# aatifjiwani/lens-flare

Hardware: AMD Instinct MI355X
Metric: Mray-surface-intersections/s + frame time, 1080p 256spp double-Gauss (higher is better)
Workload: dtype f32

## Files before the change

### lens-flare_amd/csrc/lf_api.hip

```cpp
#include <algorithm>
#include <cmath>
#include <cstdio>
#include <cstdlib>
#include <cstring>

#include "lf_internal.h"
#include "lf_march_events.h"
#include "../host/lf_collada.h"

lf_status lf_fail(const lf_ctx* ctx, lf_status st, const std::string& msg) {
  if (ctx) ctx->err = msg;
  return st;
}

static constexpr size_t kTimedCap = 512;

static hipEvent_t timing_event(lf_ctx* ctx) {
  if (!ctx->event_pool.empty()) {
    hipEvent_t e = ctx->event_pool.back();
    ctx->event_pool.pop_back();
    return e;
  }
  hipEvent_t e = nullptr;
  if (hipEventCreate(&e) != hipSuccess) return nullptr;
// ... 158 lines not shown
  ctx->lenscam_dirty = true;
  if (grow2) return lfk_mask_support(ctx);
  return LF_OK;
}

}

void lf_coat_constants(float n, float m, float np, float thickness_nm, float lambda_nm, LfCoatK* c) {
  const float m2 = m * m, n2 = n * n, np2 = np * np;
  c->dm = m2 - n2;
  c->ph = (2.0f * thickness_nm) / lambda_nm;
  c->s01 = 1.0f / (n + m);
  c->s12 = 1.0f / (m + np);
  const float q1 = std::fmaf(m2, n, n2 * m), q2 = std::fmaf(np2, m, m2 * np);
  c->p01a = m2 / q1; c->p01b = n2 / q1;
  c->p12a = np2 / q2; c->p12b = m2 / q2;
}

extern "C" {

int lf_abi_version(void) { return LF_ABI_VERSION; }

const char* lf_last_error(const lf_ctx* ctx) { return ctx ? ctx->err.c_str() : "null context"; }

static std::mutex g_knob_mu;
static std::vector<std::pair<std::string, double>> g_knob_defaults;

lf_status lf_create(lf_ctx** out, int device) {
  if (!out) return LF_ERR_INVALID;
  *out = nullptr;
  int n = 0;
  if (hipGetDeviceCount(&n) != hipSuccess || n <= 0) return LF_ERR_NO_DEVICE;
  if (device < 0 || device >= n) return LF_ERR_NO_DEVICE;
  if (hipSetDevice(device) != hipSuccess) return LF_ERR_NO_DEVICE;
  {
    hipDeviceProp_t prop;
    if (hipGetDeviceProperties(&prop, device) != hipSuccess) return LF_ERR_NO_DEVICE;
    bool any_arch = false;
#ifdef LF_EXPERIMENTS
    any_arch = std::getenv("LF_ALLOW_ANY_ARCH") != nullptr;
#endif
    if (std::strncmp(prop.gcnArchName, "gfx950", 6) != 0 && !any_arch) return LF_ERR_NO_DEVICE;
  }
  lf_ctx* ctx = new lf_ctx();
  ctx->device = device;
  if (hipStreamCreateWithFlags(&ctx->stream, hipStreamNonBlocking) != hipSuccess) {
    delete ctx;
    return LF_ERR_HIP;
  }
  ctx->own_stream = true;
#ifdef LF_EXPERIMENTS
  if (const char* sb = std::getenv("LF_MARCH_SUB_BITS")) {
    int v = std::atoi(sb);
    if (v >= 0 && v <= 8) ctx->march_sub_bits = v;
  }
#endif
  default_paraxial_lens(ctx->pl);
  bool ok = hipMalloc((void**)&ctx->flares, sizeof(LfFlares)) == hipSuccess &&
            hipMalloc((void**)&ctx->ghosts, sizeof(LfGhostList)) == hipSuccess &&
            hipMalloc((void**)&ctx->pl_dev, sizeof(LfParaxialLens)) == hipSuccess &&
            hipMalloc((void**)&ctx->lens_dev, sizeof(LfLensDev)) == hipSuccess &&
            hipMalloc((void**)&ctx->pairs_dev, sizeof(LfPairsDev)) == hipSuccess &&
            hipMalloc((void**)&ctx->counters_dev, kMarchCounterSlots * sizeof(unsigned long long)) == hipSuccess &&
            hipMalloc((void**)&ctx->scene_counters_dev, kSceneCounters * sizeof(unsigned long long)) == hipSuccess &&
            hipMalloc((void**)&ctx->primary_dev, sizeof(LfPrimaryDev)) == hipSuccess;
  for (int s = 0; s < 2 && ok; s++)
    ok = hipMalloc((void**)&ctx->ap[s].stats, sizeof(lf_aperture_stats)) == hipSuccess;
  if (!ok) { lf_destroy(ctx); return LF_ERR_OOM; }
  (void)hipMemset(ctx->flares, 0, sizeof(LfFlares));
  (void)hipMemset(ctx->ghosts, 0, sizeof(LfGhostList));
  (void)hipMemset(ctx->counters_dev, 0, kMarchCounterSlots * sizeof(unsigned long long));
  (void)hipMemset(ctx->scene_counters_dev, 0, kSceneCounters * sizeof(unsigned long long));
  if (upload_paraxial(ctx) != LF_OK) { lf_destroy(ctx); return LF_ERR_HIP; }
  {
    std::vector<std::pair<std::string, double>> defaults;
    { std::lock_guard<std::mutex> lock(g_knob_mu); defaults = g_knob_defaults; }
    for (const auto& kv : defaults) (void)lf_test_knob(ctx, kv.first.c_str(), kv.second);
  }
  *out = ctx;
  return LF_OK;
}

lf_status lf_destroy(lf_ctx* ctx) {
  if (!ctx) return LF_ERR_INVALID;
  if (ctx->comm_poisoned.load() && ctx->comm_busy.load() > 0) return LF_ERR_STATE;
  (void)hipSetDevice(ctx->device);
  (void)hipDeviceSynchronize();
  (void)lf_comm_destroy(ctx);
  if (ctx->comm_stage) (void)hipFree(ctx->comm_stage);
  free_frame_buffers(ctx);
  lf_cull_cache_free(ctx);
  for (auto& t : ctx->timed) { (void)hipEventDestroy(t.start); (void)hipEventDestroy(t.stop); }
  for (hipEvent_t e : ctx->event_pool) (void)hipEventDestroy(e);
  for (int s = 0; s < 2; s++) {
    if (ctx->ap[s].texels) (void)hipFree(ctx->ap[s].texels);
    if (ctx->ap[s].stats) (void)hipFree(ctx->ap[s].stats);
  }
  void* ptrs[] = {ctx->spectrum, ctx->twiddle, ctx->dft_rows, ctx->flares, ctx->ghosts, ctx->pl_dev,
                  ctx->lens_dev, ctx->pairs_dev, ctx->counters_dev, ctx->accum,
                  ctx->prog_dev, ctx->sun_lights_dev,
                  ctx->scene_dev.nodes, ctx->scene_dev.prims, ctx->scene_dev.normals, ctx->scene_dev.materials,
                  ctx->scene_dev.lights, ctx->env_block, ctx->probe_dev, ctx->scene_counters_dev,
                  ctx->primary_dev, ctx->cull_dev, ctx->cull_lists.list[0], ctx->cull_lists.list[1], ctx->cull_counts, ctx->cull_popc_dev,
                  ctx->tail_acc, ctx->tail_done};
  for (void* p : ptrs) if (p) (void)hipFree(p);
  if (ctx->own_stream && ctx->stream) (void)hipStreamDestroy(ctx->stream);
  delete ctx;
// ... 537 lines not shown
  LF_HIP(ctx, hipMemcpy(&f, ctx->flares, sizeof(f), hipMemcpyDeviceToHost));
  if (flare >= f.n_flares) return lf_fail(ctx, LF_ERR_INVALID, "lf_set_sun_from_flares: no such flare in the frame");
  if (!(efl_mm > 0.0)) {
    if (!paraxial_image_scale(ctx->raw_n, ctx->raw_stop, ctx->raw_radius, ctx->raw_thickness,
                              ctx->raw_ior + (size_t)(ctx->lens.n_lambda / 2) * ctx->raw_n, &efl_mm) || !(efl_mm > 0.0))
      return lf_fail(ctx, LF_ERR_INVALID, "lf_set_sun_from_flares: the prescription images no distant point on its sensor");
  }
  const double sw = ctx->sensor_w_mm, sh = sw * (double)ctx->H / (double)ctx->W;
  const float dir[3] = {(float)((f.origin[flare][0] - 0.5) * sw / efl_mm),
                        (float)((f.origin[flare][1] - 0.5) * sh / efl_mm), -1.0f};
  const float rad[3] = {(float)f.radiance[flare][0], (float)f.radiance[flare][1], (float)f.radiance[flare][2]};
  return lf_set_sun(ctx, dir, rad, angular_radius);
}

lf_status lf_set_ghost_pairs(lf_ctx* ctx, const int* pairs, int n_pairs, int include_primary) {
  if (!ctx || n_pairs < 0) return LF_ERR_INVALID;
  if (!ctx->lens_valid) return lf_fail(ctx, LF_ERR_STATE, "lf_set_ghost_pairs before lf_set_lens");
  LfPairsDev P;
  std::memset(&P, 0, sizeof(P));
  const int ns = ctx->lens.n_surf, stop = ctx->lens.stop;
  if (include_primary) { P.ij[P.n][0] = -1; P.ij[P.n][1] = -1; P.n++; }
  if (!pairs || n_pairs == 0) {
    for (int i = 0; i < ns; i++)
      for (int j = i + 1; j < ns; j++) {
        if (i == stop || j == stop) continue;
        if (P.n >= LF_MAX_PAIRS + 1) return lf_fail(ctx, LF_ERR_INVALID, "too many ghost pairs");
        P.ij[P.n][0] = i; P.ij[P.n][1] = j; P.n++;
      }
  } else {
    if (n_pairs > LF_MAX_PAIRS) return lf_fail(ctx, LF_ERR_INVALID, "too many ghost pairs");
    for (int q = 0; q < n_pairs; q++) {
      int i = pairs[2 * q], j = pairs[2 * q + 1];
      if (i == -1 && j == -1) {
        if (P.n > 0 && P.ij[0][0] < 0) return lf_fail(ctx, LF_ERR_INVALID, "primary path listed twice");
        if (P.n > 0) {
          for (int k = P.n; k > 0; k--) { P.ij[k][0] = P.ij[k - 1][0]; P.ij[k][1] = P.ij[k - 1][1]; }
        }
        P.ij[0][0] = -1; P.ij[0][1] = -1; P.n++;
        continue;
      }
      if (i < 0 || j <= i || j >= ns || i == stop || j == stop)
        return lf_fail(ctx, LF_ERR_INVALID, "ghost pair must satisfy 0 <= i < j < n, neither the stop");
      P.ij[P.n][0] = i; P.ij[P.n][1] = j; P.n++;
    }
  }
  if (P.n == 0) return lf_fail(ctx, LF_ERR_INVALID, "empty pair set");
  ctx->pairs = P;
  ctx->events_dirty = true;
  return LF_OK;
}

lf_status lf_set_pupil_subcells(lf_ctx* ctx, int bits) {
  if (!ctx) return LF_ERR_INVALID;
  if (bits < 0 || bits > 8) return lf_fail(ctx, LF_ERR_INVALID, "pupil sub-cell bits must be 0..8");
  ctx->march_sub_bits = bits;
  return LF_OK;
}

lf_status lf_set_tile_stride(lf_ctx* ctx, int stride) {
  if (!ctx) return LF_ERR_INVALID;
  if (stride != 1 && stride != 2 && stride != 4 && stride != 8)
    return lf_fail(ctx, LF_ERR_INVALID, "tile stride must be 1, 2, 4 or 8");
  ctx->march_xstride_log2 = stride == 1 ? 0 : stride == 2 ? 1 : stride == 4 ? 2 : 3;
  return LF_OK;
}

lf_status lf_trace_ghosts(lf_ctx* ctx, int spp, uint64_t key) {
  if (!ctx || spp <= 0) return LF_ERR_INVALID;
  if (!ctx->lens_valid || !ctx->sun_valid)
    return lf_fail(ctx, LF_ERR_STATE, "lf_trace_ghosts needs lf_set_lens and lf_set_sun");
  if (!ctx->ap[LF_APERTURE_STARBURST].valid)
    return lf_fail(ctx, LF_ERR_STATE, "aperture mask (LF_APERTURE_STARBURST slot) not set");
  if (ctx->pupil_target_h > 0.0f && ctx->lens.stop >= 0) {
    for (int q = 0; q < ctx->pairs.n; q++)
      if (ctx->pairs.ij[q][0] > ctx->lens.stop)
        return lf_fail(ctx, LF_ERR_STATE,
                       "a pupil target is set and the pair selection holds a pair with both mirrors behind the stop: "
                       "such pairs need the default disc (march them in a second launch, lf_set_ghost_accumulate)");
  }
  LF_HIP(ctx, hipSetDevice(ctx->device));
  lf_status st = lfk_march(ctx, spp, key);
  if (st != LF_OK) return st;
  ctx->ghost_valid = true;
  return LF_OK;
}

lf_status lf_set_march_culling(lf_ctx* ctx, int mode) {
  if (!ctx) return LF_ERR_INVALID;
  if (mode < 0 || mode > 2) return lf_fail(ctx, LF_ERR_INVALID, "march culling: 0 off, 1 on, 2 on and rebuilt at every launch");
  ctx->march_cull = mode;
  return LF_OK;
}

lf_status lf_set_cull_share(lf_ctx* ctx, int rank, int nranks) {
  if (!ctx) return LF_ERR_INVALID;
  if (nranks < 1 || nranks > 64 || rank < 0 || rank >= nranks) return lf_fail(ctx, LF_ERR_INVALID, "lf_set_cull_share: 0 <= rank < nranks <= 64");
  if (ctx->split.table == LfSplit::kComm) return lf_fail(ctx, LF_ERR_STATE, "lf_set_cull_share: the table is shared through the communicator (lf_comm_share_cull)");
  if (nranks > 1 && ctx->split.deal == LfSplit::kBlocks)
    return lf_fail(ctx, LF_ERR_STATE, "lf_set_cull_share: the frame is dealt by blocks (lf_set_block_deal): every rank builds the rows it reads, nothing is shared");
  lf_install_split(ctx, nranks > 1 ? ctx->split.with_table(LfSplit::kHost, rank, nranks) : ctx->split.with_table(LfSplit::kOwn));
  return LF_OK;
}

lf_status lf_cull_prepare(lf_ctx* ctx, int spp) {
  if (!ctx) return LF_ERR_INVALID;
  if (ctx->split.table != LfSplit::kHost) return lf_fail(ctx, LF_ERR_STATE, "lf_cull_prepare without lf_set_cull_share(rank, nranks > 1)");
  if (!ctx->lens_valid || !ctx->ap[LF_APERTURE_STARBURST].valid || ctx->W == 0)
// ... 777 lines not shown
```

### lens-flare_amd/csrc/lf_cull.hip

```cpp
#include <algorithm>
#include <cstdio>
#include <cstdlib>

#include "lf_internal.h"
#include "lf_march_events.h"
#include "lf_march_common.h"

namespace {

using namespace lfm;

constexpr int kWgWaves = 8;
constexpr int kListMax = 4096;

struct PathTally {
  unsigned long long n_rays = 0, events = 0, n_clip = 0, n_vign = 0, n_tir = 0, n_scene = 0, n_rm_lane = 0, n_rm_rows = 0;
  unsigned long long executed = 0;
  unsigned n_light = 0;
};

__device__ __forceinline__ void march_channel_factors(const LfLensDev* __restrict__ lens, float* __restrict__ s_chan, int tid) {
  if (tid < LF_MAX_LAMBDA * 3) {
    const int l = tid / 3, c = tid - 3 * l;
    s_chan[tid] = l < lens->n_lambda ? lens->sun_radiance[c] * lens->lambda_rgb[l][c] : 0.0f;
  }
}

template <int K, bool W1, int VAR>
__device__ __forceinline__ void march_started_path(const LfLensDev* __restrict__ lens, const LfPairsDev* __restrict__ pairs,
                                                   const int* __restrict__ seq_table, const LfProgRow* __restrict__ rec_table,
                                                   const LfWeightRow* __restrict__ wrec_table, const float* __restrict__ mask,
                                                   const MarchArgs& a, int q, lanemask start_mask, float X, float Y,
                                                   const StartRay& s0, int lane, int acc_slot,
                                                   unsigned long long* __restrict__ s_acc, const float* __restrict__ s_chan,
                                                   PathTally& T) {
  const int n_lambda = lens->n_lambda, prog_recs = pairs->prog_recs;
  const int n_groups = (n_lambda + K - 1) / K;
  const float inv_stop_h = a.inv_stop_h, lobe_thr = a.lobe_thr;
  const float sx = lens->sun_dir[0], sy = lens->sun_dir[1], sz = lens->sun_dir[2];
  const float inv_1mc = lens->sun_inv_one_minus_cos, sun_ss = lens->sun_ss;
  const int n_ev = pairs->ev_cnt[q];
  const int* const seq = seq_table + pairs->ev_off[q];
  for (int g = 0; g < n_groups; g++) {
    const LfProgRow* const recs = rec_table + (size_t)g * (size_t)prog_recs;
    const LfWeightRow* const wrecs = wrec_table + (size_t)g * (size_t)prog_recs;
    Ray r[K];
    lanemask alive[K];
    unsigned nlive = 0u;
#pragma unroll
    for (int j = 0; j < K; j++) {
      r[j] = Ray{X, Y, 0.0f, fmaf(X, X, Y * Y), s0.dx, s0.dy, s0.dz, s0.w0, 1.0f};
      const float ns = lens->n_start[min(g * K + j, n_lambda - 1)];
      r[j].dx *= ns; r[j].dy *= ns; r[j].dz *= ns;
      alive[j] = (g * K + j < n_lambda) ? start_mask : 0ull;
      nlive += (unsigned)__popcll(alive[j]);
    }
    T.n_rays += nlive;
    unsigned ev32 = 0u;
    unsigned se = (unsigned)*(const int __attribute__((address_space(4)))*)(seq);
    int e = 0;
    if (n_ev > 0 && nlive != 0u) for (;;) {
      const unsigned cur = se;
      se = (unsigned)*(const int __attribute__((address_space(4)))*)(seq + e + 1);
      const LfProgRow wr = load_prec(recs, cur & 0xffffu);
      LfWeightRow ww;
      if (W1) ww = load_wrec(wrecs, cur & 0xffffu);
// ... 22 lines not shown
          for (int j = 0; j < K; j++) {
            if (K > 1 && __builtin_expect(alive[j] == 0ull, 0)) { okv[j] = 0ull; gv[j] = 0ull; continue; }
            okv[j] = surface_event<W1>(r[j], wr.dzv, wr.curv, wr.ch, wr.c2, wr.sc, wr.cn22[j], wr.rn2[j],
                                       wr.delta[j], wr.h2, false, false, wr.sgn, gv[j], ww.fs[j], ww.fo[j], ww.fi[j],
                                       CoatSel<VAR>{wrec_table, ww.coat, j});
            died |= alive[j] & ~okv[j];
          }
        } else if (kind == (unsigned)LF_EV_REFLECT) {
#pragma unroll
          for (int j = 0; j < K; j++) {
            if (K > 1 && __builtin_expect(alive[j] == 0ull, 0)) { okv[j] = 0ull; gv[j] = 0ull; continue; }
            okv[j] = surface_event<W1>(r[j], wr.dzv, wr.curv, wr.ch, wr.c2, wr.sc, wr.cn22[j], wr.rn2[j],
                                       wr.delta[j], wr.h2, true, false, wr.sgn, gv[j], ww.fs[j], ww.fo[j], ww.fi[j],
                                       CoatSel<VAR>{wrec_table, ww.coat, j});
            died |= alive[j] & ~okv[j];
          }
        } else {
#pragma unroll
          for (int j = 0; j < K; j++) {
            if (K > 1 && __builtin_expect(alive[j] == 0ull, 0)) { okv[j] = 0ull; gv[j] = 0ull; continue; }
            okv[j] = surface_event<W1>(r[j], wr.dzv, wr.curv, wr.ch, wr.c2, wr.sc, wr.cn22[j], wr.rn2[j],
                                       wr.delta[j], wr.h2, (kind & LF_EV_REFLECT) != 0, (kind & LF_EV_FLAT) != 0,
                                       wr.sgn, gv[j], ww.fs[j], ww.fo[j], ww.fi[j],
                                       CoatSel<VAR>{wrec_table, ww.coat, j});
            died |= alive[j] & ~okv[j];
          }
        }
        if (__builtin_expect(died != 0ull, 0)) {
#pragma unroll
          for (int j = 0; j < K; j++) {
            T.n_vign += (unsigned)__popcll(alive[j] & ~gv[j]);
            T.n_tir += (unsigned)__popcll(alive[j] & gv[j] & ~okv[j]);
            nlive -= (unsigned)__popcll(alive[j] & ~okv[j]);
            alive[j] &= okv[j];
          }
          if (nlive == 0u) e = n_ev;
        }
      }
      ev32 += nlive;
      if (++e >= n_ev) break;
    }
    T.events += ev32;
    T.executed += ev32;
    if (nlive == 0u) continue;
    T.n_scene += nlive;
    lanemask lit[K], lit_any = 0ull;
#pragma unroll
    for (int j = 0; j < K; j++) {
      const float cg = fmaf(r[j].dx, sx, fmaf(r[j].dy, sy, r[j].dz * sz));
      lit[j] = alive[j] & __ballot(cg > lobe_thr);
      lit_any |= lit[j];
    }
    if (lit_any == 0ull) continue;
    for (int j = 0; j < K; j++) {
      lanemask lj = lit[0];
#pragma unroll
      for (int jj = 1; jj < K; jj++) lj = (j == jj) ? lit[jj] : lj;
      if (lj == 0ull) continue;
      const int l = g * K + j;
      Ray rw = j == 0 ? r[0] : j == 1 ? r[K > 1 ? 1 : 0] : r[K > 2 ? 2 : 0];
      if (!W1) {
        rw = Ray{X, Y, 0.0f, fmaf(X, X, Y * Y), s0.dx, s0.dy, s0.dz, s0.w0, 1.0f};
        { const float ns = lens->n_start[l]; rw.dx *= ns; rw.dy *= ns; rw.dz *= ns; }
        T.n_rm_lane += (unsigned long long)((unsigned)n_ev * (unsigned)__popcll(lj));
        T.n_rm_rows += (unsigned)n_ev;
        weighted_remarch<VAR>(rw, seq, n_ev, j, recs, wrecs, wrec_table, mask, inv_stop_h, a.mw, a.mh);
      }
      const float qq = lobe_q(rw.dx, rw.dy, rw.dz, sx, sy, sz, sun_ss, inv_1mc);
      const float om = 1.0f - qq;
      float contrib = __fdiv_rn(rw.wn, rw.wd) * (om * om);
      contrib = (((lj >> lane) & 1ull) != 0ull && qq < 1.0f && contrib > 0.0f) ? contrib : 0.0f;
      T.n_light += contrib > 0.0f ? 1u : 0u;
#pragma unroll
      for (int c = 0; c < 3; c++) {
        const float v = contrib * s_chan[l * 3 + c];
        const unsigned long long fx = (unsigned long long)(v * 68719476736.0f);
        if (fx) atomicAdd(&s_acc[acc_slot * 3 + c], fx);
      }
    }
  }
}

template <int K, bool REFLECT, bool FLAT>
__device__ __forceinline__ lanemask surface_rows(Ray (&r)[K], const lanemask (&alive)[K], const LfProgRow& wr, lanemask (&okv)[K],
                                                 lanemask (&gv)[K]) {
  lanemask died = 0ull;
#pragma unroll
  for (int j = 0; j < K; j++) {
    if (K > 1 && __builtin_expect(alive[j] == 0ull, 0)) { okv[j] = 0ull; gv[j] = 0ull; continue; }
    okv[j] = surface_event<false>(r[j], wr.dzv, wr.curv, wr.ch, wr.c2, wr.sc, wr.cn22[j], wr.rn2[j], wr.delta[j], wr.h2,
                                  REFLECT, FLAT, wr.sgn, gv[j]);
    died |= alive[j] & ~okv[j];
  }
  return died;
}

template <int K, int VAR>
__device__ __forceinline__ void march_started_set(const LfLensDev* __restrict__ lens, const LfPairsDev* __restrict__ pairs,
                                                  const int* __restrict__ seq_table, const LfProgRow* __restrict__ rec_table,
                                                  const LfWeightRow* __restrict__ wrec_table, const float* __restrict__ mask,
                                                  const MarchArgs& a, unsigned long long todo, lanemask active_mask, float X, float Y,
                                                  const StartRay& s0, int lane, unsigned long long* __restrict__ s_acc,
                                                  const int2* __restrict__ s_meta, const float* __restrict__ s_chan,
                                                  PathTally& T) {
  const int n_lambda = lens->n_lambda, prog_recs = pairs->prog_recs;
  const int n_groups = (n_lambda + K - 1) / K;
// ... 40 lines not shown
          pn = nlive; forked = true;
          ev_logical = (unsigned long long)seg * mult; ev_exec = seg; seg = 0u; mult = 1u;
        }
        const unsigned cur = se;
        se = (unsigned)*(const int __attribute__((address_space(4)))*)(seq + e + 1);
        const LfProgRow wr = load_prec(recs, cur & 0xffffu);
        const unsigned kind = cur >> 16;
        lanemask okv[K], gv[K], died = 0ull;
        if (__builtin_expect(kind == 0u, 1)) {
          died = surface_rows<K, false, false>(r, alive, wr, okv, gv);
        } else if (kind & LF_EV_STOP) {
#pragma unroll
          for (int j = 0; j < K; j++) {
            if (K > 1 && __builtin_expect(alive[j] == 0ull, 0)) { okv[j] = 0ull; gv[j] = 0ull; continue; }
            okv[j] = stop_event_var<false, VAR>(r[j], wr.dzv, wr.h2, inv_stop_h, mask, a.mw, a.mh);
            gv[j] = okv[j];
            died |= alive[j] & ~okv[j];
          }
        } else if (kind & LF_EV_REFLECT) {
          if (kind & LF_EV_FLAT) died = surface_rows<K, true, true>(r, alive, wr, okv, gv);
          else died = surface_rows<K, true, false>(r, alive, wr, okv, gv);
        } else {
          died = surface_rows<K, false, true>(r, alive, wr, okv, gv);
        }
        if (__builtin_expect(died != 0ull, 0)) {
          const bool stop_row = (kind & LF_EV_STOP) != 0;
#pragma unroll
          for (int j = 0; j < K; j++) {
            const unsigned nd = (unsigned)__popcll(alive[j] & ~okv[j]);
            const unsigned nv = (unsigned)__popcll(alive[j] & ~gv[j]);
            T.n_clip += stop_row ? (unsigned long long)nd * mult : 0ull;
            T.n_vign += stop_row ? 0ull : (unsigned long long)nv * mult;
            T.n_tir += stop_row ? 0ull : (unsigned long long)(nd - nv) * mult;
            nlive -= nd;
            alive[j] &= okv[j];
          }
          if (nlive == 0u) e = n_ev;
        }
        seg += nlive;
        if (++e >= n_ev) break;
      }
      T.events += ev_logical + (unsigned long long)seg * mult;
      T.executed += ev_exec + seg;
      if (!forked && L < n_ev) break;
      if (nlive != 0u) {
        T.n_scene += nlive;
        lanemask lit[K], lit_any = 0ull;
#pragma unroll
        for (int j = 0; j < K; j++) {
          const float cg = fmaf(r[j].dx, sx, fmaf(r[j].dy, sy, r[j].dz * sz));
          lit[j] = alive[j] & __ballot(cg > lobe_thr);
          lit_any |= lit[j];
        }
        if (lit_any != 0ull) {
          for (int j = 0; j < K; j++) {
            lanemask lj = lit[0];
#pragma unroll
            for (int jj = 1; jj < K; jj++) lj = (j == jj) ? lit[jj] : lj;
            if (lj == 0ull) continue;
            const int l = g * K + j;
            Ray rw = Ray{X, Y, 0.0f, fmaf(X, X, Y * Y), s0.dx, s0.dy, s0.dz, s0.w0, 1.0f};
            { const float ns = lens->n_start[l]; rw.dx *= ns; rw.dy *= ns; rw.dz *= ns; }
            T.n_rm_lane += (unsigned long long)((unsigned)n_ev * (unsigned)__popcll(lj));
            T.n_rm_rows += (unsigned)n_ev;
            weighted_remarch<VAR>(rw, seq, n_ev, j, recs, wrecs, wrec_table, mask, inv_stop_h, a.mw, a.mh);
            const float qq = lobe_q(rw.dx, rw.dy, rw.dz, sx, sy, sz, sun_ss, inv_1mc);
            const float om = 1.0f - qq;
            float contrib = __fdiv_rn(rw.wn, rw.wd) * (om * om);
            contrib = (((lj >> lane) & 1ull) != 0ull && qq < 1.0f && contrib > 0.0f) ? contrib : 0.0f;
            T.n_light += contrib > 0.0f ? 1u : 0u;
#pragma unroll
            for (int c = 0; c < 3; c++) {
              const float v = contrib * s_chan[l * 3 + c];
              const unsigned long long fx = (unsigned long long)(v * 68719476736.0f);
              if (fx) atomicAdd(&s_acc[lane * 3 + c], fx);
            }
          }
        }
      }
      if (!forked || left == 0ull) break;
#pragma unroll
      for (int j = 0; j < K; j++) { r[j] = p[j]; alive[j] = palive[j]; }
      nlive = pn;
      depth = L;
    }
  }
}

#ifndef LF_SHARED_WAVES
#define LF_SHARED_WAVES 6
#endif
template <int K, bool W1, int MODE, int VAR>
__global__ __launch_bounds__(64 * kWgWaves, (K == 1 ? 8 : MODE == 1 ? LF_SHARED_WAVES : 6))
void k_march_cull(const LfLensDev* __restrict__ lens, const LfPairsDev* __restrict__ pairs,
                  const int* __restrict__ seq_table, const LfProgRow* __restrict__ rec_table,
                  const LfWeightRow* __restrict__ wrec_table, const float* __restrict__ mask, MarchArgs a,
                  LfCullArgs cull, double* __restrict__ ghost, unsigned long long* __restrict__ accum,
                  unsigned long long* __restrict__ counters) {
  __shared__ unsigned long long s_acc[64 * 3];
  __shared__ unsigned long long s_cnt[kMarchCounters];
  __shared__ int s_next, s_nlist;
  __shared__ unsigned short s_list[kListMax];
  __shared__ int2 s_meta[MODE == 1 ? kCullMaxPaths : 1];
  __shared__ float s_chan[LF_MAX_LAMBDA * 3];
  const int tid = threadIdx.x;
  if (tid < 64 * 3) s_acc[tid] = 0ull;
  march_channel_factors(lens, s_chan, tid);
  if (tid < kMarchCounters) s_cnt[tid] = 0ull;
  if (tid == 0) { s_next = 0; s_nlist = 0; }
  if (MODE == 1 && tid < pairs->n && tid < kCullMaxPaths) {
    const int n_ev = pairs->ev_cnt[tid], i1 = pairs->ij[tid][0];
    s_meta[tid] = make_int2((n_ev << 16) | (i1 < 0 ? n_ev : lens->n_surf - 1 - i1), pairs->ev_off[tid]);
  }
  __syncthreads();

  const int tiles_x = ((a.W + (8 << a.xs) - 1) >> (3 + a.xs)) << a.xs;
#ifdef LF_EXPERIMENTS
  if (cull.wg_clock && tid == 0) cull.wg_clock[2 * (size_t)blockIdx.x] = wall_clock64();
  struct ClockAtExit { unsigned long long* p; __device__ ~ClockAtExit() { if (p && threadIdx.x == 0) *p = wall_clock64(); } }
      clock_at_exit{cull.wg_clock ? cull.wg_clock + 2 * (size_t)blockIdx.x + 1 : nullptr};
#endif
  const unsigned n_head = (unsigned)a.tail_from * (unsigned)a.sgroups;
  const bool tail = a.tail_groups > 1 && blockIdx.x >= n_head;
  const int sgroups = tail ? a.tail_groups : a.sgroups;
  const int sg = tail ? (int)((blockIdx.x - n_head) % (unsigned)sgroups) : (int)(blockIdx.x % (unsigned)sgroups);
  const unsigned slot = tail ? (unsigned)a.tail_from + (blockIdx.x - n_head) / (unsigned)sgroups : blockIdx.x / (unsigned)sgroups;
  const int tile_lin = (int)((slot & ~63u) | ((slot & 7u) << 3) | ((slot >> 3) & 7u));
  if (tile_lin >= a.n_tiles) return;
  int tx, trow;
  march_tile_of(a, tile_lin, tiles_x, tx, trow);
  const unsigned tile_id = (unsigned)(trow * tiles_x + tx);
  const int wave = __builtin_amdgcn_readfirstlane(tid >> 6);
  const int lane = tid & 63;
  const int x = ((tx >> a.xs) << (3 + a.xs)) + ((lane & 7) << a.xs) + (tx & ((1 << a.xs) - 1)), y = trow * 8 + (lane >> 3);
  const bool active = x < a.W && y >= a.y0 && y < a.y1;
  const lanemask active_mask = __ballot(active);
  const unsigned p = (unsigned)y * (unsigned)a.W + (unsigned)x;
  const int blk = ((trow * 8) >> cull.blk_log2) * cull.blocks_x + ((((tx >> a.xs) << (3 + a.xs))) >> cull.blk_log2);
  const unsigned long long* const crow = cull.table + lf_cull_row_of_block(blk, cull.share_n, cull.share_nb) * (size_t)(cull.cells + 1);
  const int blk_lane = (min(y, a.H - 1) >> cull.blk_log2) * cull.blocks_x + (min(x, a.W - 1) >> cull.blk_log2);
  const unsigned long long* const crow_lane = cull.multi ? cull.table + lf_cull_row_of_block(blk_lane, cull.share_n, cull.share_nb) * (size_t)(cull.cells + 1) : crow;

  const float pitch = lens->pitch, pupil_h = lens->pupil_h, geom_norm = lens->geom_norm;
  const float half_w = a.half_w, half_h = a.half_h, vz_u = a.vz;
  const int GG = a.G * a.G;
  const bool per_lane = (1 << a.sub_bits) < cull.m;

  PathTally T;

  const int n_mine = (a.spp - sg + sgroups - 1) / sgroups;
  for (int chunk0 = 0; chunk0 < n_mine; chunk0 += kListMax) {
    const int chunk_n = min(kListMax, n_mine - chunk0);
    for (int k = tid; k < chunk_n; k += 64 * kWgWaves) {
      const int s = sg + (chunk0 + k) * sgroups;
      bool work = true;
      if (s >= GG && !cull.multi) work = crow[cull.cells] != 0ull;
      if (s < GG && !per_lane && !cull.multi) {
        const uint4 r2 = philox4x32_10(make_uint4(tile_id, (unsigned)s, kDomainSubcell, 0u), a.key);
        const unsigned sxi = a.sub_bits ? (r2.x >> (32 - a.sub_bits)) : 0u, syi = a.sub_bits ? (r2.y >> (32 - a.sub_bits)) : 0u;
        const int cy = s / a.G, cx = s - cy * a.G;
        work = crow[(cy * cull.m + (int)((syi << cull.m_shift) >> a.sub_bits)) * cull.P + cx * cull.m + (int)((sxi << cull.m_shift) >> a.sub_bits)] != 0ull;
      }
      if (work) s_list[atomicAdd(&s_nlist, 1)] = (unsigned short)k;
    }
    __syncthreads();
    const int n_list = s_nlist;
    for (;;) {
      int k = 0;
      if (lane == 0) k = atomicAdd(&s_next, 1);
      k = __builtin_amdgcn_readfirstlane(k);
      if (k >= n_list) break;
      const int s = sg + (chunk0 + (int)s_list[k]) * sgroups;
      const uint4 rnd = philox4x32_10(make_uint4(p, (unsigned)s, kDomainMarch, 0u), a.key);
      const float jx = u01(rnd.x), jy = u01(rnd.y);
      float ua = u01(rnd.z), ub = u01(rnd.w);
      int entry = -1;
      if (s < GG) {
        const int cy = s / a.G, cx = s - cy * a.G;
        const uint4 r2 = philox4x32_10(make_uint4(tile_id, (unsigned)s, kDomainSubcell, 0u), a.key);
        const unsigned sxi = a.sub_bits ? (r2.x >> (32 - a.sub_bits)) : 0u;
        const unsigned syi = a.sub_bits ? (r2.y >> (32 - a.sub_bits)) : 0u;
        ua = ((float)cx + ((float)sxi + ua) * a.inv_sub) * a.inv_G;
        ub = ((float)cy + ((float)syi + ub) * a.inv_sub) * a.inv_G;
        if (!per_lane) entry = (cy * cull.m + (int)((syi << cull.m_shift) >> a.sub_bits)) * cull.P + cx * cull.m + (int)((sxi << cull.m_shift) >> a.sub_bits);
      }
      if (s >= GG) entry = cull.cells;
      const float pa0 = fmaf(2.0f, ua, -1.0f), pb0 = fmaf(2.0f, ub, -1.0f);
      const float X = -(((float)x + jx) - half_w) * pitch;
      const float Y = -(((float)y + jy) - half_h) * pitch;
      if (MODE == 1) {
        const unsigned long long todo = crow[entry];
        if (todo == 0ull) continue;
        const StartRay s0 = aim_at_pupil(X, Y, pa0, pb0, pupil_h, vz_u, geom_norm);
        march_started_set<K, VAR>(lens, pairs, seq_table, rec_table, wrec_table, mask, a, todo, active_mask, X, Y, s0, lane, s_acc, s_meta, s_chan, T);
        continue;
      }
      unsigned long long mine, todo;
      if (entry >= 0 && !cull.multi) { todo = crow[entry]; mine = todo; }
      else {
        const int fx = min(cull.P - 1, (int)(ua * (float)cull.P)), fy = min(cull.P - 1, (int)(ub * (float)cull.P));
        mine = active ? crow_lane[entry >= 0 ? entry : fy * cull.P + fx] : 0ull;
        unsigned lo = (unsigned)mine, hi = (unsigned)(mine >> 32);
        for (int off = 32; off > 0; off >>= 1) { lo |= __shfl_xor(lo, off); hi |= __shfl_xor(hi, off); }
        todo = ((unsigned long long)__builtin_amdgcn_readfirstlane(hi) << 32) | (unsigned long long)__builtin_amdgcn_readfirstlane(lo);
      }
      if (todo == 0ull) continue;
      const StartRay s0 = aim_at_pupil(X, Y, pa0, pb0, pupil_h, vz_u, geom_norm);
      unsigned long long left_q = todo;
      while (left_q != 0ull) {
        const int q = __builtin_ctzll(left_q);
        left_q &= left_q - 1ull;
        const lanemask start_mask = active_mask & __ballot(((mine >> q) & 1ull) != 0ull);
        march_started_path<K, W1, VAR>(lens, pairs, seq_table, rec_table, wrec_table, mask, a, q, start_mask, X, Y, s0, lane, lane, s_acc, s_chan, T);
      }
    }
    __syncthreads();
    if (tid == 0) { s_next = 0; s_nlist = 0; }
    __syncthreads();
  }

  {
    unsigned long long v6 = T.n_light;
    for (int off = 32; off > 0; off >>= 1) v6 += __shfl_down(v6, off);
    const unsigned long long vals[kMarchCounters] = {T.n_rays, T.events, T.n_clip, T.n_vign, T.n_tir, T.n_scene, v6, T.executed, T.n_rm_lane, T.n_rm_rows};
    if (lane == 0) {
#pragma unroll
      for (int i = 0; i < kMarchCounters; i++)
        if (vals[i]) atomicAdd(&s_cnt[i], vals[i]);
    }
  }
  __syncthreads();
  if (wave == 0 && lane < kMarchCounters && s_cnt[lane]) atomicAdd(&counters[lane], s_cnt[lane]);

  if (tail) {
// ... 329 lines not shown
```

### lens-flare_amd/csrc/lf_internal.h

```cpp
#pragma once

#include <hip/hip_runtime.h>

#include <atomic>
#include <cmath>
#include <cstdint>
#include <mutex>
#include <string>
#include <vector>

#include "lensflare.h"

constexpr int kMarchCounters = 10;
constexpr int kMarchCounterSlots = 256;
constexpr int kMarchHistSlot = 16;
constexpr int kMarchPairSlot = 64;
constexpr int kMaxParaxialGhosts = 3 * 105;
constexpr int kMaxGhostTris = 2 * kMaxParaxialGhosts;

struct LfFlares {
  int n_flares;
  float angle_to_sun;
  double origin[LF_MAX_FLARES][2];
  double radiance[LF_MAX_FLARES][3];
// ... 93 lines not shown
  float curv, h2, eta;
  float sgn;
  int flags;
  float radius;
  float eta2;
  float n_in, n_out;
  int surf_dir;
  int pad[5];
};
enum { LF_EV_REFLECT = 1, LF_EV_STOP = 2, LF_EV_FLAT = 4 };
struct alignas(16) LfProgHdr {
  int flags;
  int skip;
  int rec;
  int rec_next;
};
struct alignas(64) LfProgRow {
  float dzv, curv, h2, sc;
  float sgn;
  float delta[3];
  float cn22[3];
  float ch;
  float rn2[3];
  float c2;
};
struct alignas(64) LfWeightRow {
  float fs[3], pad0;
  float fo[3], pad1;
  float fi[3], pad2;
  int coat;
  float pad3[3];
};
struct alignas(32) LfCoatK {
  float dm, ph, s01, s12, p01a, p01b, p12a, p12b;
};
struct LfCoatings {
  int n = 0;
  float lambda_nm[LF_MAX_LAMBDA] = {};
  float thickness_nm[LF_MAX_SURFACES] = {};
  float index[LF_MAX_LAMBDA * LF_MAX_SURFACES] = {};
};
constexpr float kCoatMaxThicknessNm = 10000.0f;
void lf_coat_constants(float n_in, float m, float n_out, float thickness_nm, float lambda_nm, LfCoatK* c);
enum { LF_EV_REST1 = 8, LF_EV_SAVE0 = 0x10, LF_EV_SAVE1 = 0x20, LF_EV_END = 0x40, LF_EV_REST0 = 0x80 };

constexpr int kCullBlockLog2 = 6;
constexpr double kCullBigBlockMm = 1.25;
constexpr int kCullMaxPaths = 64;
constexpr double kCullMaxBlockMm = 1.8;
constexpr int kCullOcc = 32;
__host__ __device__ inline size_t lf_cull_row_of_block(int b, int share_n, int share_nb) {
  return share_n > 1 ? (size_t)(b % share_n) * (size_t)share_nb + (size_t)(b / share_n) : (size_t)b;
}
struct LfCullArgs {
  const unsigned long long* table;
  int blocks_x, blocks_y;
  int prefix_ok;
  int multi;
  int share_n, share_nb;
  int blk_log2;
  int cells;
  int P, m, m_shift;
  unsigned long long* tail_acc;
  int* tail_done;
  int items_chunk0;
#ifdef LF_EXPERIMENTS
  unsigned long long* wg_clock;
#endif
};

constexpr int kDealBlockLog2 = 6;
struct LfDeal { int n, rank, bx; };
__host__ __device__ inline bool lf_deal_mine(const LfDeal& d, int x, int y) {
  if (d.n <= 1) return true;
  return d.bx > 0 ? ((y >> kDealBlockLog2) * d.bx + (x >> kDealBlockLog2)) % d.n == d.rank : (y >> 3) % d.n == d.rank;
}
struct LfSplit {
  enum Deal { kRows, kBlocks } deal = kRows;
  int rank = 0, n = 1;
  enum Table { kOwn, kComm, kHost } table = kOwn;
  int table_rank = 0, table_n = 1;
  LfSplit with_deal(Deal d, int r, int k) const { LfSplit s = *this; s.deal = d; s.rank = r; s.n = k; return s; }
  LfSplit with_table(Table t, int r = 0, int k = 1) const { LfSplit s = *this; s.table = t; s.table_rank = r; s.table_n = k; return s; }
};
struct LfCullLists { unsigned* list[2] = {nullptr, nullptr}; size_t cap[2] = {0, 0}; };
struct LfCullSlab { int rank = 0, n = 1, nb = 0; bool own_rows_only = false; };
struct LfCullCache {
  uint64_t key = 0;
  bool reused = false;
  int n_levels = 0;
  int levels[8] = {};
  unsigned n_mine = 0;
  unsigned* slots = nullptr;
  size_t slot_off[8] = {};
  float* foots[8] = {};
  size_t n_foot[8] = {};
  size_t bytes = 0;
  bool thrash = false;
  uint64_t last_key = 0;
  uint64_t nofit_key = 0;
  double nofit_mb = 0.0;
};

struct LfPrimaryRow {
  float dzv, curv, ch, c2, sc, h2;
  int kind;
// ... 276 lines not shown
```

### lens-flare_amd/csrc/lf_march.hip

```cpp
#include <algorithm>
#include <cmath>
#include <cstdio>
#include <cstdlib>
#include <vector>
#include <cstring>
#include <utility>

#include "lf_internal.h"
#include "lf_march_events.h"
#include "lf_march_common.h"

namespace {

using namespace lfm;



__device__ __forceinline__ void park(float2* __restrict__ slot, int lane, const Ray& r) {
  slot[lane] = make_float2(r.px, r.py);
  slot[64 + lane] = make_float2(r.hz, r.dx);
  slot[128 + lane] = make_float2(r.dy, r.dz);
}
__device__ __forceinline__ void unpark(const float2* __restrict__ slot, int lane, Ray& r) {
  const float2 a = slot[lane], b = slot[64 + lane], c = slot[128 + lane];
// ... 312 lines not shown
                                          cur.delta[j], cur.h2, (fl & LF_EV_REFLECT) != 0,
                                          (fl & LF_EV_FLAT) != 0, cur.sgn, gv[j] LF_WROW_ARGS(j));
              died |= alive[j] & ~okv[j];
            }
            if (__builtin_expect(died != 0ull, 0)) {
#pragma unroll
              for (int j = 0; j < K; j++) {
                vign32 += mult * (unsigned)__popcll(alive[j] & ~gv[j]);
                tir32 += mult * (unsigned)__popcll(alive[j] & gv[j] & ~okv[j]);
                nlive -= (unsigned)__popcll(alive[j] & ~okv[j]);
                alive[j] &= okv[j];
              }
              dead = nlive == 0u;
            }
            const unsigned live = nlive;
            ev32 += mult * live;
            exec32 += live;
            endfl = fl;
            sk = hdr.skip;
            step();
          }
          if (dead) {
            e = e - kHdr + (((unsigned)sk & ~3u) << 2);
            hdr = load_phdr(prog, e);
            cur = load_prec(recs, (unsigned)hdr.rec);
            LF_WROW_LOAD((unsigned)hdr.rec);
            if ((sk & 3) == 1) unpark_all(1, alive1);
            else if ((sk & 3) == 2) unpark_all(0, alive0);
          } else if (endfl & LF_EV_END) {
            scene32 += nlive;
            lanemask lit[K], lit_any = 0ull;
#pragma unroll
            for (int j = 0; j < K; j++) {
              const float cg = fmaf(r[j].dx, sx, fmaf(r[j].dy, sy, r[j].dz * sz));
              lit[j] = alive[j] & __ballot(cg > lobe_thr);
              lit_any |= lit[j];
              LF_PAIR_STAT(0, endfl >> 24, alive[j] != 0ull ? 1u : 0u);
              LF_PAIR_STAT(1, endfl >> 24, lit[j] != 0ull ? 1u : 0u);
              LF_PAIR_STAT(2, endfl >> 24, (unsigned)__popcll(lit[j]));
            }
#ifdef LF_MARCH_LIT_MAP
            if (lit_any != 0ull && g_lit_map[0] != nullptr && lane_id() == 0) {
              const int bx64 = (tx >> a.xs) << (3 + a.xs) >> 6, trow_ = trow;
              const int nbx = (a.W + 63) >> 6;
              const int blkA = ((trow_ * 8) >> 6) * nbx + bx64, blkB = trow_ * nbx + bx64;
              for (int m = 0; m < 4; m++) {
                const int P = 16 << m;
                const int fx = min(P - 1, (int)(lm_u * (float)P)), fy = min(P - 1, (int)(lm_v * (float)P));
                atomicOr(&g_lit_map[m][((size_t)blkA * P + fy) * P + fx], 1ull << (endfl >> 24));
                atomicOr(&g_lit_map[4 + m][((size_t)blkB * P + fy) * P + fx], 1ull << (endfl >> 24));
              }
            }
#endif
            if (lit_any != 0ull) {
              const int q = (int)(endfl >> 24);
              for (int j = 0; j < K; j++) {
                lanemask lj = lit[0];
#pragma unroll
                for (int jj = 1; jj < K; jj++) lj = (j == jj) ? lit[jj] : lj;
                if (lj == 0ull) continue;
                const int l = g * K + j;
                const int* __restrict__ w = seq_table + pairs->ev_off[q];
                const int lo = launder(lane);
                Ray rw{LF_START(0, lo), LF_START(1, lo), 0.0f, 0.0f, LF_START(2, lo),
                       LF_START(3, lo), LF_START(4, lo), LF_START(5, lo), 1.0f};
                rw.r2 = fmaf(rw.px, rw.px, rw.py * rw.py);
                { const float ns = lens->n_start[l]; rw.dx *= ns; rw.dy *= ns; rw.dz *= ns; }
                if (kW1) {
                  rw = j == 0 ? r[0] : j == 1 ? r[K > 1 ? 1 : 0] : r[K > 2 ? 2 : 0];
                } else {
                n_rm_lane += (unsigned long long)((unsigned)pairs->ev_cnt[q] * (unsigned)__popcll(lj));
                n_rm_rows += (unsigned)pairs->ev_cnt[q];
                for (int left = pairs->ev_cnt[q]; left > 0; --left, ++w) {
                  const unsigned se = (unsigned)*(const int __attribute__((address_space(4)))*)(w);
                  const LfProgRow wr = load_prec(recs, se & 0xffffu);
                  const LfWeightRow ww = load_wrec(wrecs, se & 0xffffu);
                  const unsigned wfl = se >> 16;
                  const float w_cn22 = j == 0 ? wr.cn22[0] : j == 1 ? wr.cn22[1] : wr.cn22[2];
                  const float w_rn2 = j == 0 ? wr.rn2[0] : j == 1 ? wr.rn2[1] : wr.rn2[2];
                  const float w_delta = j == 0 ? wr.delta[0] : j == 1 ? wr.delta[1] : wr.delta[2];
                  const float w_fs = j == 0 ? ww.fs[0] : j == 1 ? ww.fs[1] : ww.fs[2];
                  const float w_fo = j == 0 ? ww.fo[0] : j == 1 ? ww.fo[1] : ww.fo[2];
                  const float w_fi = j == 0 ? ww.fi[0] : j == 1 ? ww.fi[1] : ww.fi[2];
                  if (wfl & LF_EV_STOP) {
                    (void)stop_event_var<true, VAR>(rw, wr.dzv, wr.h2, inv_stop_h, mask, a.mw, a.mh);
                  } else {
                    lanemask geom_ok;
                    (void)surface_event<true>(rw, wr.dzv, wr.curv, wr.ch, wr.c2, wr.sc, w_cn22, w_rn2, w_delta, wr.h2,
                                              (wfl & LF_EV_REFLECT) != 0, (wfl & LF_EV_FLAT) != 0, wr.sgn, geom_ok,
                                              w_fs, w_fo, w_fi, CoatSel<VAR>{wrec_table, ww.coat, j});
                  }
                }
                }
                const float qq = lobe_q(rw.dx, rw.dy, rw.dz, sx, sy, sz, sun_ss, inv_1mc);
                const float om = 1.0f - qq;
                float contrib = __fdiv_rn(rw.wn, rw.wd) * (om * om);
                contrib = (((lj >> lane) & 1ull) != 0ull && qq < 1.0f && contrib > 0.0f) ? contrib : 0.0f;
                n_light += contrib > 0.0f ? 1u : 0u;
#pragma unroll
                for (int c = 0; c < 3; c++) {
                  const float v = contrib * (lens->sun_radiance[c] * lens->lambda_rgb[l][c]);
                                    const unsigned long long fx = (unsigned long long)(v * 68719476736.0f);
                  if (fx) atomicAdd(&s_acc[lane * 3 + c], fx);
                }
              }
            }
// ... 766 lines not shown
```

### lens-flare_amd/csrc/lf_march_common.h

```cpp
#pragma once

#include <cstddef>

#include "lf_internal.h"
#include "lf_march_events.h"

namespace lfm {

__device__ __forceinline__ float lobe_q(float dx, float dy, float dz, float sx, float sy, float sz,
                                        float ss, float inv_1mc) {
  const float cg = fmaf(dx, sx, fmaf(dy, sy, dz * sz));
  const float cx = fmaf(dy, sz, -(dz * sy)), cy = fmaf(dz, sx, -(dx * sz)), cz = fmaf(dx, sy, -(dy * sx));
  const float c2 = fmaf(cx, cx, fmaf(cy, cy, cz * cz));
  const float dd = fmaf(dx, dx, fmaf(dy, dy, dz * dz));
  const float ds = dd * ss;
  const float den = fmaf(lf_sqrt(ds), cg, ds);
  return __fdiv_rn(c2, den) * inv_1mc;
}

struct MarchArgs {
  int mw, mh, W, H, y0, y1;
  int spp, G;
  float inv_G;
  int sub_bits;
  float inv_sub;
  int trow0, tperiod;
  LfDeal deal;
  int sgroups;
  int tail_from, tail_groups;
  uint2 key;
  float inv_stop_h;
  float half_w, half_h;
  float vz;
  float lobe_thr;
  int accumulate;
  int n_tiles;
  int xs;
};

__device__ __forceinline__ void march_tile_of(const MarchArgs& a, int tile_lin, int tiles_x, int& tx, int& trow) {
  if (a.deal.bx > 0) {
    const int b = a.deal.rank + (tile_lin >> 6) * a.deal.n, w = tile_lin & 63;
    const int by = b / a.deal.bx;
    trow = by * 8 + (w >> 3);
    tx = (b - by * a.deal.bx) * 8 + (w & 7);
  } else {
    const int tj = tile_lin / tiles_x;
    tx = tile_lin - tj * tiles_x;
    trow = a.trow0 + tj * a.tperiod;
  }
}
__device__ __forceinline__ bool march_owns(const MarchArgs& a, int x, int y) {
  if (a.deal.bx > 0) return lf_deal_mine(a.deal, x, y);
  const int t = y >> 3;
  return t >= a.trow0 && (t - a.trow0) % a.tperiod == 0;
}

typedef int lf_i16 __attribute__((ext_vector_type(16)));
typedef int lf_i4 __attribute__((ext_vector_type(4)));
typedef const lf_i16 __attribute__((address_space(4))) * lf_const_prow_ptr;
typedef const lf_i4 __attribute__((address_space(4))) * lf_const_phdr_ptr;
__device__ __forceinline__ LfProgRow load_prec(const LfProgRow* __restrict__ base, unsigned off) {
  typedef const char __attribute__((address_space(4))) * cptr;
  const lf_i16 v = *(lf_const_prow_ptr)((cptr)(base) + off);
  LfProgRow r;
  r.dzv = __int_as_float(v[0]); r.curv = __int_as_float(v[1]); r.h2 = __int_as_float(v[2]);
  r.sc = __int_as_float(v[3]); r.sgn = __int_as_float(v[4]);
#pragma unroll
  for (int j = 0; j < 3; j++) {
    r.delta[j] = __int_as_float(v[5 + j]); r.cn22[j] = __int_as_float(v[8 + j]); r.rn2[j] = __int_as_float(v[12 + j]);
// ... 64 lines not shown
```

Baseline: 929,300.

## Gate weighted remarch on exact lobe test and carry sub-cell draws in cull list

```diff
diff --git a/lens-flare_amd/csrc/lf_api.hip b/lens-flare_amd/csrc/lf_api.hip
--- a/lens-flare_amd/csrc/lf_api.hip
+++ b/lens-flare_amd/csrc/lf_api.hip
@@ -234,7 +234,7 @@
 #ifdef LF_EXPERIMENTS
   if (const char* sb = std::getenv("LF_MARCH_SUB_BITS")) {
     int v = std::atoi(sb);
-    if (v >= 0 && v <= 8) ctx->march_sub_bits = v;
+    if (v >= 0 && v <= kMaxSubcellBits) ctx->march_sub_bits = v;
   }
 #endif
   default_paraxial_lens(ctx->pl);
@@ -878,7 +878,7 @@
 
 lf_status lf_set_pupil_subcells(lf_ctx* ctx, int bits) {
   if (!ctx) return LF_ERR_INVALID;
-  if (bits < 0 || bits > 8) return lf_fail(ctx, LF_ERR_INVALID, "pupil sub-cell bits must be 0..8");
+  if (bits < 0 || bits > kMaxSubcellBits) return lf_fail(ctx, LF_ERR_INVALID, "pupil sub-cell bits must be 0..8");
   ctx->march_sub_bits = bits;
   return LF_OK;
 }
diff --git a/lens-flare_amd/csrc/lf_cull.hip b/lens-flare_amd/csrc/lf_cull.hip
--- a/lens-flare_amd/csrc/lf_cull.hip
+++ b/lens-flare_amd/csrc/lf_cull.hip
@@ -11,7 +11,8 @@
 using namespace lfm;
 
 constexpr int kWgWaves = 8;
-constexpr int kListMax = 4096;
+constexpr int kListBits = 12;
+constexpr int kListMax = 1 << kListBits;
 
 struct PathTally {
   unsigned long long n_rays = 0, events = 0, n_clip = 0, n_vign = 0, n_tir = 0, n_scene = 0, n_rm_lane = 0, n_rm_rows = 0;
@@ -140,6 +141,10 @@
       lit_any |= lit[j];
     }
     if (lit_any == 0ull) continue;
+    if (!W1) {
+      lit_any = lobe_gate<K>(r, lit, sx, sy, sz, sun_ss, inv_1mc);
+      if (lit_any == 0ull) continue;
+    }
     for (int j = 0; j < K; j++) {
       lanemask lj = lit[0];
 #pragma unroll
@@ -286,6 +291,7 @@
           lit[j] = alive[j] & __ballot(cg > lobe_thr);
           lit_any |= lit[j];
         }
+        if (lit_any != 0ull) lit_any = lobe_gate<K>(r, lit, sx, sy, sz, sun_ss, inv_1mc);
         if (lit_any != 0ull) {
           for (int j = 0; j < K; j++) {
             lanemask lj = lit[0];
@@ -334,7 +340,8 @@
   __shared__ unsigned long long s_acc[64 * 3];
   __shared__ unsigned long long s_cnt[kMarchCounters];
   __shared__ int s_next, s_nlist;
-  __shared__ unsigned short s_list[kListMax];
+  static_assert(2 * kMaxSubcellBits <= 32 - kListBits, "a listed sample's sub-cell does not fit beside its place in the chunk");
+  __shared__ unsigned s_list[kListMax];
   __shared__ int2 s_meta[MODE == 1 ? kCullMaxPaths : 1];
   __shared__ float s_chan[LF_MAX_LAMBDA * 3];
   const int tid = threadIdx.x;
@@ -388,14 +395,18 @@
     for (int k = tid; k < chunk_n; k += 64 * kWgWaves) {
       const int s = sg + (chunk0 + k) * sgroups;
       bool work = true;
+      unsigned drawn = 0u;
       if (s >= GG && !cull.multi) work = crow[cull.cells] != 0ull;
-      if (s < GG && !per_lane && !cull.multi) {
+      if (s < GG) {
         const uint4 r2 = philox4x32_10(make_uint4(tile_id, (unsigned)s, kDomainSubcell, 0u), a.key);
         const unsigned sxi = a.sub_bits ? (r2.x >> (32 - a.sub_bits)) : 0u, syi = a.sub_bits ? (r2.y >> (32 - a.sub_bits)) : 0u;
-        const int cy = s / a.G, cx = s - cy * a.G;
-        work = crow[(cy * cull.m + (int)((syi << cull.m_shift) >> a.sub_bits)) * cull.P + cx * cull.m + (int)((sxi << cull.m_shift) >> a.sub_bits)] != 0ull;
-      }
-      if (work) s_list[atomicAdd(&s_nlist, 1)] = (unsigned short)k;
+        drawn = sxi | (syi << kMaxSubcellBits);
+        if (!per_lane && !cull.multi) {
+          const int cy = s / a.G, cx = s - cy * a.G;
+          work = crow[(cy * cull.m + (int)((syi << cull.m_shift) >> a.sub_bits)) * cull.P + cx * cull.m + (int)((sxi << cull.m_shift) >> a.sub_bits)] != 0ull;
+        }
+      }
+      if (work) s_list[atomicAdd(&s_nlist, 1)] = (unsigned)k | (drawn << kListBits);
     }
     __syncthreads();
     const int n_list = s_nlist;
@@ -404,16 +415,16 @@
       if (lane == 0) k = atomicAdd(&s_next, 1);
       k = __builtin_amdgcn_readfirstlane(k);
       if (k >= n_list) break;
-      const int s = sg + (chunk0 + (int)s_list[k]) * sgroups;
+      const unsigned listed = (unsigned)__builtin_amdgcn_readfirstlane((int)s_list[k]);
+      const int s = sg + (chunk0 + (int)(listed & (unsigned)(kListMax - 1))) * sgroups;
       const uint4 rnd = philox4x32_10(make_uint4(p, (unsigned)s, kDomainMarch, 0u), a.key);
       const float jx = u01(rnd.x), jy = u01(rnd.y);
       float ua = u01(rnd.z), ub = u01(rnd.w);
       int entry = -1;
       if (s < GG) {
         const int cy = s / a.G, cx = s - cy * a.G;
-        const uint4 r2 = philox4x32_10(make_uint4(tile_id, (unsigned)s, kDomainSubcell, 0u), a.key);
-        const unsigned sxi = a.sub_bits ? (r2.x >> (32 - a.sub_bits)) : 0u;
-        const unsigned syi = a.sub_bits ? (r2.y >> (32 - a.sub_bits)) : 0u;
+        const unsigned sxi = (listed >> kListBits) & ((1u << kMaxSubcellBits) - 1u);
+        const unsigned syi = listed >> (kListBits + kMaxSubcellBits);
         ua = ((float)cx + ((float)sxi + ua) * a.inv_sub) * a.inv_G;
         ub = ((float)cy + ((float)syi + ub) * a.inv_sub) * a.inv_G;
         if (!per_lane) entry = (cy * cull.m + (int)((syi << cull.m_shift) >> a.sub_bits)) * cull.P + cx * cull.m + (int)((sxi << cull.m_shift) >> a.sub_bits);
diff --git a/lens-flare_amd/csrc/lf_internal.h b/lens-flare_amd/csrc/lf_internal.h
--- a/lens-flare_amd/csrc/lf_internal.h
+++ b/lens-flare_amd/csrc/lf_internal.h
@@ -169,6 +169,7 @@
 __host__ __device__ inline size_t lf_cull_row_of_block(int b, int share_n, int share_nb) {
   return share_n > 1 ? (size_t)(b % share_n) * (size_t)share_nb + (size_t)(b / share_n) : (size_t)b;
 }
+constexpr int kMaxSubcellBits = 8;
 struct LfCullArgs {
   const unsigned long long* table;
   int blocks_x, blocks_y;
diff --git a/lens-flare_amd/csrc/lf_march.hip b/lens-flare_amd/csrc/lf_march.hip
--- a/lens-flare_amd/csrc/lf_march.hip
+++ b/lens-flare_amd/csrc/lf_march.hip
@@ -388,6 +388,7 @@
               }
             }
 #endif
+            if (!kW1 && lit_any != 0ull) lit_any = lobe_gate<K>(r, lit, sx, sy, sz, sun_ss, inv_1mc);
             if (lit_any != 0ull) {
               const int q = (int)(endfl >> 24);
               for (int j = 0; j < K; j++) {
diff --git a/lens-flare_amd/csrc/lf_march_common.h b/lens-flare_amd/csrc/lf_march_common.h
--- a/lens-flare_amd/csrc/lf_march_common.h
+++ b/lens-flare_amd/csrc/lf_march_common.h
@@ -16,6 +16,18 @@
   const float ds = dd * ss;
   const float den = fmaf(lf_sqrt(ds), cg, ds);
   return __fdiv_rn(c2, den) * inv_1mc;
+}
+
+template <int K>
+__device__ __forceinline__ lanemask lobe_gate(const Ray (&r)[K], lanemask (&lit)[K], float sx, float sy, float sz, float ss,
+                                              float inv_1mc) {
+  lanemask lit_any = 0ull;
+#pragma unroll
+  for (int j = 0; j < K; j++) {
+    if (lit[j] != 0ull) lit[j] &= __ballot(lobe_q(r[j].dx, r[j].dy, r[j].dz, sx, sy, sz, ss, inv_1mc) < 1.0f);
+    lit_any |= lit[j];
+  }
+  return lit_any;
 }
 
 struct MarchArgs {
```

Measured after the change: 948,700 (median of 6 runs). 2.1% higher.
